# stein7/nerf-navigation

Measured on AMD Instinct MI355X. Metric: ray-samples/sec, Stonehenge-class 800x800 novel-view render, higher is better.
Workload: dtype f16

## Files before the change

### nerf-navigation_amd/csrc/render_fused.hip

```cpp
#include "ngp_mlp.h"
#include "ngp_sh.h"
#include "ngp_field.h"
#include "ngp_march.h"
#include "ngp_camera.h"

__global__ void k_field_forward_lds(rf_params P, const float* __restrict__ xyzs, const float* __restrict__ dirs, uint32_t M,
                                    float* __restrict__ sigmas, void* __restrict__ rgbs, bool rgb_half);

static int rf_field_forward(const ngp_field_t* field_host, const float* xyzs, const float* dirs, uint32_t M, float* sigmas, void* rgbs, bool rgb_half, void* stream) {
    rf_params P;
    int rc = rf_fill_params("field_forward", field_host, P);
    if (rc != NGP_OK) return rc;
    if (M == 0) return NGP_OK;
    NGP_REQUIRE(xyzs && dirs && sigmas && rgbs, "field_forward: null pointer");
    const uint32_t npairs = (M + 31) >> 5;
    uint32_t blocks = ngp_div_up(npairs, RF_BLOCK / 64);
    if (blocks > 256 * RF_FIELD_WG_PER_CU) blocks = 256 * RF_FIELD_WG_PER_CU;
    hipLaunchKernelGGL(k_field_forward_lds, dim3(blocks), dim3(RF_BLOCK), 36 * 1024, (hipStream_t)stream, P, xyzs, dirs, M, sigmas, rgbs, rgb_half);
    NGP_CHECK_LAUNCH("field_forward");
    return NGP_OK;
}

extern "C" int ngp_field_forward(const ngp_field_t* field_host, const float* xyzs, const float* dirs, uint32_t M,
                                 float* sigmas, float* rgbs, void* stream) {
    return rf_field_forward(field_host, xyzs, dirs, M, sigmas, rgbs, false, stream);
}

extern "C" int ngp_field_forward_half(const ngp_field_t* field_host, const float* xyzs, const float* dirs, uint32_t M,
                                      float* sigmas, void* rgbs_half, void* stream) {
    return rf_field_forward(field_host, xyzs, dirs, M, sigmas, rgbs_half, true, stream);
}


#ifndef RV_S
#define RV_S 12
#endif
static_assert(RV_S >= 2, "RV_S must be at least 2: the one-sample-per-round frame kernel has been removed");
#ifndef RV_BANDS
#define RV_BANDS 32u
#endif
#ifndef RV_REFILL_MIN
#define RV_REFILL_MIN 64
#endif
#ifndef RV_SLAB_STEPS
#define RV_SLAB_STEPS 16
#endif
#ifndef RV_BLOCK_THREADS
#define RV_BLOCK_THREADS 512
#endif
#ifndef RV_BLOCKS_PER_CU
#define RV_BLOCKS_PER_CU 1
#endif
static constexpr uint32_t RV_BLOCK = RV_BLOCK_THREADS;
static constexpr int RV_WAVES_PER_SIMD = (RV_BLOCK_THREADS / 256) * RV_BLOCKS_PER_CU;
static constexpr int RV_WAVES = RV_BLOCK / 64;
static constexpr uint32_t RV_LDS_W = RV_NFRAG * 1024;
static constexpr uint32_t RV_LDS_SH = RV_WAVES * 64 * 32;
static constexpr uint32_t RV_LDS_LV = 4 * 96;

struct rf_frame {
    const float* rays_o; const float* rays_d; uint32_t N;
    ngp_camera cam;
    const ngp_camera* cams; uint32_t frame_rays;
    float aabb[6]; float min_near;
    const uint8_t* bitfield; uint32_t C, H;
    float dt_gamma; uint32_t max_steps;
    float bg[3];
    float* image; float* depth; float* weights_sum;
    uint32_t* stats; uint32_t* queue;
#ifdef RV_COUNTERS
    uint32_t* hist;
#endif
    const uint32_t* coarse;
    uint32_t coarse_words;
    uint32_t tile_w;
    uint32_t skip;
    const uint32_t* occ_ext;
    float occ_unit, occ_top;
    const uint32_t* tile_perm;
};

__global__ __launch_bounds__(256) void k_build_coarse(const uint8_t* __restrict__ bitfield, uint32_t n_blocks_total,
                                                      uint32_t* __restrict__ coarse, uint32_t blocks_per_level, uint32_t C, uint32_t* __restrict__ ext) {
    const uint32_t w = blockIdx.x * 256 + threadIdx.x;
    if (w * 32 >= n_blocks_total) return;
    const uint64_t* b64 = reinterpret_cast<const uint64_t*>(bitfield);
    uint32_t bits = 0;
    #pragma unroll 8
    for (uint32_t i = 0; i < 32; i++) {
        const uint32_t blk = w * 32 + i;
        if (blk < n_blocks_total && b64[blk] != 0ull) bits |= 1u << i;
    }
    coarse[w] = bits;
    if (ext && bits) {
        uint32_t nb = 1;
        while (nb * nb * nb < blocks_per_level) nb <<= 1;
        uint32_t lo[3] = {0xFFFFFFFFu, 0xFFFFFFFFu, 0xFFFFFFFFu}, hi[3] = {0u, 0u, 0u};
        const uint32_t words_per_level = blocks_per_level / 32u, level = w / words_per_level;
        ngp_occ_extent_word(bits, w - level * words_per_level, level, C, nb, lo, hi);
        #pragma unroll
        for (int k = 0; k < 3; k++) { atomicMax(ext + k, (1u << 20) - lo[k]); atomicMax(ext + 3 + k, hi[k]); }
    }
}

struct rv_ray { float ox, oy, oz, dx, dy, dz, rdx, rdy, rdz; };
struct rv_consts {
    float bound, rbound, dt_gamma, dt_min, dt_max, rH, H3, Hf, Cf, Hm1;
    const uint8_t* grid;
    __device__ __forceinline__ int mip(int e) const { return (int)fminf(Cf - 1.0f, fmaxf(0.0f, (float)e)); }
};
__device__ __forceinline__ float rv_uniform(float v) {
    return __builtin_bit_cast(float, __builtin_amdgcn_readfirstlane(__builtin_bit_cast(int, v)));
}
struct rv_view : rv_ray, rv_consts {
    __device__ __forceinline__ rv_view(const rv_ray& r, const rv_consts& k) : rv_ray(r), rv_consts(k) {}
};

typedef ngp_point<rv_view> rv_point;

struct rv_block_cache { uint32_t blk = 0xffffffffu, lo = 0, hi = 0; };

struct rv_tested { rv_point r; bool maybe; uint32_t sw; };

__device__ __forceinline__ bool rv_test(const rv_view& m, const uint32_t* __restrict__ lds_coarse, uint32_t coarse_words, rv_block_cache& bc,
                                        float tc, rv_tested& st
#ifdef RV_COUNTERS
                                        , int* rv_dbg_ptr
#endif
                                        ) {
    rv_point& r = st.r;
    r.at(m, tc);
    const uint32_t mort = ngp_morton3((uint32_t)r.nx, (uint32_t)r.ny, (uint32_t)r.nz);
    st.maybe = true;
    st.sw = 0;
    if (lds_coarse) {
        const uint32_t blk = mort >> 6;
        st.maybe = (lds_coarse[(uint32_t)r.level * coarse_words + (blk >> 5)] >> (blk & 31u)) & 1u;
        st.sw = (uint32_t)r.level * coarse_words + ((blk >> 6) << 1);
#ifdef RV_COUNTERS
        *rv_dbg_ptr = st.maybe ? 0 : ((lds_coarse[st.sw] | lds_coarse[st.sw + 1]) == 0u ? 2 : 1);
#endif
    }
    if (!st.maybe) return false;
    if (lds_coarse) {
        const uint32_t gblk = (uint32_t)r.level * (coarse_words << 5) + (mort >> 6);
        if (gblk != bc.blk) {
            const uint2 w = reinterpret_cast<const uint2*>(m.grid)[gblk];
            bc.blk = gblk; bc.lo = w.x; bc.hi = w.y;
        }
        return (((mort & 32u) ? bc.hi : bc.lo) >> (mort & 31u)) & 1u;
    }
    const uint32_t index = (uint32_t)((float)r.level * m.H3 + (float)mort);
    return (m.grid[index >> 3] >> (index & 7u)) & 1u;
}

__device__ __forceinline__ float rv_leave(const rv_view& m, const uint32_t* __restrict__ lds_coarse, float M, const rv_tested& st, float tc) {
    const rv_point& r = st.r;
    const float tt = r.cell_exit(m, tc);
    if (lds_coarse && !st.maybe) {
        const int sh = ((lds_coarse[st.sw] | lds_coarse[st.sw + 1]) == 0u) ? 4 : 2;
        const float ta = ngp_try_skip(m, r, tc, tt, sh, M);
        if (ta >= 0.0f) return ta;
    }
    float tp;
    return ngp_advance(m, tc, tt, tp);
}

__device__ __forceinline__ bool rv_probe(const rv_ray& ray, const rv_consts& k, const uint32_t* __restrict__ lds_coarse, uint32_t coarse_words,
                                         float M, rv_block_cache& bc, float& t, float& x, float& y, float& z, float& dt
#ifdef RV_COUNTERS
                                         , int* rv_dbg_ptr
#endif
                                         ) {
    const rv_view m(ray, k);
    rv_tested st;
#ifdef RV_COUNTERS
    const bool occ = rv_test(m, lds_coarse, coarse_words, bc, t, st, rv_dbg_ptr);
#else
    const bool occ = rv_test(m, lds_coarse, coarse_words, bc, t, st);
#endif
    x = st.r.x; y = st.r.y; z = st.r.z; dt = st.r.dt;
    if (occ) return true;
    t = rv_leave(m, lds_coarse, M, st, t);
    return false;
}


template <bool FIXED>
__device__ __forceinline__ void rf_points_loop(const rf_params& P, const rf_iter_class cls_rt, const rf_lane_levels& lv, const ngp_h8* __restrict__ lds_w,
                                               const float* __restrict__ xyzs, const float* __restrict__ dirs, uint32_t M,
                                               float* __restrict__ sigmas, void* __restrict__ rgbs_v, bool rgb_half) {
    const rf_iter_class cls = FIXED ? rf_iter_class{1u, 12u, 2u} : cls_rt;
    const int lane = threadIdx.x & 63, g = lane >> 4, s = lane & 15;
    const uint32_t wave = (blockIdx.x * RF_BLOCK + threadIdx.x) >> 6, nwaves = gridDim.x * (RF_BLOCK / 64);
    const uint32_t npairs = (M + 31) >> 5;
    for (uint32_t pair = wave; pair < npairs; pair += nwaves) {
        ngp_h8 x[2];
        ngp_h4 shq[2];
        uint32_t m[2];
        #pragma unroll
        for (int n = 0; n < 2; n++) {
            m[n] = pair * 32 + 16 * n + s;
            const uint64_t mm = m[n] < M ? m[n] : 0;
            const float px = xyzs[3 * mm], py = xyzs[3 * mm + 1], pz = xyzs[3 * mm + 2];
            float sh[16];
            sh_eval<4>(dirs[3 * mm], dirs[3 * mm + 1], dirs[3 * mm + 2], P.shn, sh);
            #pragma unroll
            for (int j = 0; j < 4; j++) {
                float v = sh[j];
                if (g == 1) v = sh[4 + j];
                if (g == 2) v = sh[8 + j];
                if (g == 3) v = sh[12 + j];
                shq[n][j] = ngp_f2h(v);
            }
            x[n] = rf_encode<false>(P, lv, cls, px, py, pz);
        }
        float sg[2], cr[2], cg[2], cb[2];
        rv_mlp_tiles<2>(lds_w, lane, x, shq, sg, cr, cg, cb);
        #pragma unroll
        for (int n = 0; n < 2; n++)
            if (g == 0 && m[n] < M) {
                rv_activate(P, sg[n], cr[n], cg[n], cb[n]);
                sigmas[m[n]] = sg[n];
                if (rgb_half) {
                    _Float16* rgbs = static_cast<_Float16*>(rgbs_v);
                    rgbs[3ull * m[n]] = (_Float16)cr[n]; rgbs[3ull * m[n] + 1] = (_Float16)cg[n]; rgbs[3ull * m[n] + 2] = (_Float16)cb[n];
                } else {
                    float* rgbs = static_cast<float*>(rgbs_v);
                    rgbs[3ull * m[n]] = cr[n]; rgbs[3ull * m[n] + 1] = cg[n]; rgbs[3ull * m[n] + 2] = cb[n];
                }
            }
    }
}

__global__ __launch_bounds__(RF_BLOCK, RF_FIELD_WG_PER_CU) void k_field_forward_lds(rf_params P, const float* __restrict__ xyzs, const float* __restrict__ dirs,
                                                                    uint32_t M, float* __restrict__ sigmas, void* __restrict__ rgbs, bool rgb_half) {
    extern __shared__ __attribute__((aligned(16))) unsigned char rf_smem[];
    ngp_h8* lds_w = reinterpret_cast<ngp_h8*>(rf_smem);
    const int lane = threadIdx.x & 63, g = lane >> 4, wave = threadIdx.x >> 6;
    rv_stage_weights(P, lds_w, wave, RF_BLOCK / 64, lane);
    rf_lane_levels lv;
    rf_setup_levels(P, g, lv);
    __syncthreads();
    const rf_iter_class cls = rf_classify(lv);
    if (cls.dense == 1u && cls.select == 2u && cls.hashed == 12u) rf_points_loop<true>(P, cls, lv, lds_w, xyzs, dirs, M, sigmas, rgbs, rgb_half);
    else rf_points_loop<false>(P, cls, lv, lds_w, xyzs, dirs, M, sigmas, rgbs, rgb_half);
}

__device__ __forceinline__ void rv_ray_od(const rf_frame& F, uint32_t ray, float o[3], float d[3]) {
    if (F.rays_o) {
        #pragma unroll
        for (int k = 0; k < 3; k++) { o[k] = F.rays_o[3ull * ray + k]; d[k] = F.rays_d[3ull * ray + k]; }
    } else if (F.cams) {
        const uint32_t f = ray / F.frame_rays;
        const ngp_camera c = F.cams[f];
        o[0] = c.t[0]; o[1] = c.t[1]; o[2] = c.t[2];
        ngp_camera_ray(c, ray - f * F.frame_rays, d);
    } else {
        o[0] = F.cam.t[0]; o[1] = F.cam.t[1]; o[2] = F.cam.t[2];
        ngp_camera_ray(F.cam, ray, d);
    }
}

__device__ __forceinline__ uint32_t rv_ray_of(uint32_t idx, uint32_t tile_w) {
    if (tile_w == 0) return idx;
    const uint32_t tile = idx >> 6, in = idx & 63u, tiles_x = tile_w >> 3;
    const uint32_t ty = tile / tiles_x, tx = tile - ty * tiles_x;
    const uint32_t p = in >> 4, s = in & 15u;
    const uint32_t px = (p & 1u) * 4 + (s & 3u), py = (p >> 1) * 4 + (s >> 2);
    return (ty * 8 + py) * tile_w + tx * 8 + px;
}

static constexpr uint32_t RV_LDS_SMP = RV_WAVES * 64 * RV_S * 16;

template <bool FIXED>
__device__ __forceinline__ void rv_frame_loop(const rf_params& P, const rf_frame& F, const rf_iter_class cls_rt,
                                              const ngp_h8* __restrict__ lds_w, _Float16* lds_sh, const rf_lane_levels* lds_lv,
                                              float4* lds_smp, const uint32_t* lds_coarse, const float* lds_occ) {
    const rf_iter_class cls = FIXED ? rf_iter_class{1u, 12u, 2u} : cls_rt;
    const int lane = threadIdx.x & 63, g = lane >> 4, s = lane & 15, wave = threadIdx.x >> 6;
    const int wave_s = __builtin_amdgcn_readfirstlane(wave);

    _Float16* my_sh = lds_sh + (wave * 64 + lane) * 16;
    const _Float16* wave_sh = lds_sh + wave * 64 * 16;
    float4* my_smp = lds_smp + (wave * 64 + lane) * RV_S;
    float4* wave_smp = lds_smp + wave * 64 * RV_S;

    rv_consts K;
    K.bound = P.bound; K.rbound = rv_uniform(1.0f / P.bound); K.dt_gamma = F.dt_gamma;
    K.Hf = rv_uniform((float)F.H); K.Cf = rv_uniform((float)F.C); K.Hm1 = rv_uniform((float)(F.H - 1));
    K.rH = rv_uniform(1.0f / K.Hf);
    K.H3 = rv_uniform((float)(F.H * F.H * F.H));
    K.dt_min = rv_uniform((2.0f * 1.7320508075688772f) / (float)F.max_steps);
    K.dt_max = rv_uniform(((2.0f * 1.7320508075688772f) * (float)(1 << (F.C - 1))) / K.Hf);
    K.grid = F.bitfield;

    bool active = false;
    uint32_t ray = 0, nsamp = 0;
    rv_ray m;
    float t = 0, last_t = 0, near = 0, far = 0;
    float ws = 0, dacc = 0, cr = 0, cg = 0, cb = 0, tcomp = 0;
    bool exhausted = false;
    uint32_t rv_q = blockIdx.x & 7u, rv_q_seen = 0;
    rv_block_cache bc;
    uint32_t n_samples_local = 0, n_tiles = 0, n_capped_local = 0, n_hit_local = 0;
#ifdef RV_COUNTERS
    uint32_t n_rounds = 0, n_trips = 0, n_probe[4] = {0, 0, 0, 0};
    unsigned long long c_refill = 0, c_march = 0, c_tiles = 0, c_comp = 0;
    const unsigned long long c_start = __builtin_readcyclecounter();
    unsigned long long c_last = c_start;
#define RV_TICK(acc) { const unsigned long long c_now = __builtin_readcyclecounter(); acc += c_now - c_last; c_last = c_now; }
    uint32_t* rv_hist = F.hist;
    unsigned long long rv_t0 = 0;
    if (rv_hist) {
        unsigned long long* p0 = reinterpret_cast<unsigned long long*>(F.queue + 24);
        const unsigned long long now = wall_clock64();
        const unsigned long long old = atomicCAS(p0, 0ull, now);
        rv_t0 = __shfl(old ? old : now, 0, 64);
    }
#else
#define RV_TICK(acc)
#endif

    for (;;) {
        if (!exhausted) {
            const unsigned long long need = __ballot(!active);
            if (need && (uint32_t)__popcll(need) >= RV_REFILL_MIN) {
                const uint32_t cnt = (uint32_t)__popcll(need);
                uint32_t base = 0;
                const uint32_t n_tiles64 = (F.N + 63u) >> 6;
                const uint32_t q_lo = (uint32_t)(((unsigned long long)n_tiles64 * rv_q) / RV_BANDS) << 6;
                uint32_t q_hi = (uint32_t)(((unsigned long long)n_tiles64 * (rv_q + 1u)) / RV_BANDS) << 6;
                q_hi = q_hi < F.N ? q_hi : F.N;
                if (lane == 0) base = atomicAdd(F.queue + 32 + rv_q, cnt);
                base = __shfl(base, 0, 64) + q_lo;
                if (!active) {
                    const uint32_t idx = base + (uint32_t)__popcll(need & ((1ull << lane) - 1ull));
                    if (idx < q_hi) {
                        ray = rv_ray_of(F.tile_perm ? (F.tile_perm[idx >> 6] << 6) | (idx & 63u) : idx, F.tile_w);
                        float o[3], d[3];
                        rv_ray_od(F, ray, o, d);
                        ngp_near_far_inline(o, d, F.aabb, F.min_near, near, far);
                        if (lds_occ) {
                            float n2, f2;
                            ngp_near_far_inline(o, d, lds_occ, 0.0f, n2, f2);
                            far = f2 == 3.402823466e+38f ? near : fminf(far, f2 + lds_occ[6]);
                        }
                        m.ox = o[0]; m.oy = o[1]; m.oz = o[2];
                        m.dx = d[0]; m.dy = d[1]; m.dz = d[2];
                        m.rdx = 1.0f / m.dx; m.rdy = 1.0f / m.dy; m.rdz = 1.0f / m.dz;
                        t = near; last_t = near; tcomp = near;
                        ws = 0; dacc = 0; cr = 0; cg = 0; cb = 0; nsamp = 0;
                        float sh[16];
                        sh_eval<4>(m.dx, m.dy, m.dz, P.shn, sh);
                        #pragma unroll
                        for (int j = 0; j < 16; j++) my_sh[j] = ngp_f2h(sh[j]);
                        active = true;
                    }
                }
                if (base + cnt >= q_hi) {
                    rv_q += 8u;
                    if (rv_q >= RV_BANDS) rv_q = (rv_q + 1u) & 7u;
                    if (++rv_q_seen == RV_BANDS) exhausted = true;
                }
            }
        }
        if (__ballot(active) == 0ull) {
            if (exhausted) break;
            continue;
        }
        RV_TICK(c_refill)

        int cnt = 0;
        bool ended = false;
#ifdef RV_COUNTERS
        n_rounds++;
        const unsigned long long rv_live = __ballot(active);
#endif
        {
            rv_ray mr = m;
            float far_r = far;
            asm("" : "+v"(mr.ox), "+v"(mr.oy), "+v"(mr.oz), "+v"(mr.dx), "+v"(mr.dy), "+v"(mr.dz),
                     "+v"(mr.rdx), "+v"(mr.rdy), "+v"(mr.rdz), "+v"(far_r));
            rv_consts Kr = K;
            asm("" : "+v"(Kr.Hf), "+v"(Kr.Hm1), "+v"(Kr.Cf), "+v"(Kr.rH), "+v"(Kr.dt_min), "+v"(Kr.dt_max), "+v"(Kr.rbound), "+v"(Kr.H3));
            const float M = (active && F.skip) ? ngp_skip_margin(mr, K.bound, lds_occ ? far_r + 4.0f * K.bound : far_r) : __builtin_inff();
            const uint32_t slot0 = ((uint32_t)wave_s * 64u + __builtin_amdgcn_mbcnt_hi(~0u, __builtin_amdgcn_mbcnt_lo(~0u, 0u))) * RV_S;
            float4* const smp_w = lds_smp + slot0;
            int probes = 0;
            float t_lim = __builtin_inff();
            auto march = [&](int upto) {
                for (;;) {
#ifdef RV_COUNTERS
                    n_trips = __builtin_amdgcn_readfirstlane(n_trips) + 1;
#endif
                    if (!(t < far_r && nsamp < F.max_steps)) { ended = true; break; }
                    if (RV_SLAB_STEPS > 0 && !(t < t_lim)) break;
                    float x, y, z, dt;
#ifdef RV_COUNTERS
                    int pc = 0;
                    const bool hit = rv_probe(mr, Kr, lds_coarse, F.coarse_words, M, bc, t, x, y, z, dt, &pc);
                    n_probe[pc]++;
                    if (hit) {
#else
                    if (rv_probe(mr, Kr, lds_coarse, F.coarse_words, M, bc, t, x, y, z, dt)) {
#endif
                        smp_w[cnt] = make_float4(x, y, z, t);
                        t += dt;
                        nsamp++;
                        if (++cnt >= upto) break;
                    }
                    if (++probes >= RF_PROBES_PER_ROUND) break;
                }
            };
            if (RV_SLAB_STEPS > 0) {
                if (active) march(1);
                const float t_first = cnt ? smp_w[0].w : __builtin_inff();
                float tf = t_first;
                #pragma unroll
                for (int off = 1; off < 64; off <<= 1) tf = fminf(tf, __shfl_xor(tf, off, 64));
                t_lim = tf + (float)RV_SLAB_STEPS * K.dt_min;
                if (cnt && !(t_first < t_lim)) { t = t_first; nsamp--; cnt = 0; ended = false; }
                if (active && cnt && !ended) march(RV_S);
            } else if (active) {
                march(RV_S);
            }
        }

        __builtin_amdgcn_fence(__ATOMIC_RELEASE, "wavefront");
        __builtin_amdgcn_wave_barrier();
        __builtin_amdgcn_fence(__ATOMIC_ACQUIRE, "wavefront");

        RV_TICK(c_march)
        int col_src;
        {
            uint32_t rank = 0, above = 0;
            const uint32_t below_me = __builtin_amdgcn_mbcnt_hi(~0u, __builtin_amdgcn_mbcnt_lo(~0u, 0u));
            #pragma unroll
            for (int c = RV_S; c >= 0; c--) {
                const unsigned long long mc = __ballot(cnt == c);
                if (cnt == c) rank = above + (uint32_t)__popcll(mc & ((1ull << below_me) - 1ull));
                above += (uint32_t)__popcll(mc);
            }
            col_src = __builtin_amdgcn_ds_permute((int)(rank << 2), (int)below_me);
        }
        #pragma unroll 1
        for (int p = 0; p < 4; p++) {
            const int src = __shfl(col_src, 16 * p + s, 64);
            const int ccol = __shfl(cnt, src, 64);
            if (__ballot(ccol > 0) == 0ull) continue;
            const ngp_h4 shq = *reinterpret_cast<const ngp_h4*>(wave_sh + src * 16 + 4 * g);
            const rf_lane_levels lv = lds_lv[g];
            #pragma unroll 1
            for (int k = 0; k < RV_S; k += 2) {
                if (__ballot(ccol > k) == 0ull) break;
                if (k + 1 < RV_S && __ballot(ccol > k + 1) != 0ull) {
                    ngp_h8 xs[2];
                    #pragma unroll
                    for (int n = 0; n < 2; n++) {
                        float4 q = wave_smp[src * RV_S + k + n];
                        if (!(ccol > k + n)) q = make_float4(0.f, 0.f, 0.f, 0.f);
                        xs[n] = rf_encode<true>(P, lv, cls, q.x, q.y, q.z);
                    }
                    n_tiles += 2;
                    const ngp_h4 ss[2] = {shq, shq};
                    float a[2], b[2], c[2], d[2];
                    rv_mlp_tiles<2>(lds_w, lane, xs, ss, a, b, c, d);
                    #pragma unroll
                    for (int n = 0; n < 2; n++)
                        if (g == 0 && ccol > k + n) {
                            ngp_h4 r;
                            r[0] = (_Float16)a[n]; r[1] = (_Float16)b[n]; r[2] = (_Float16)c[n]; r[3] = (_Float16)d[n];
                            *reinterpret_cast<ngp_h4*>(&wave_smp[src * RV_S + k + n]) = r;
                        }
                } else {
                    float4 q = wave_smp[src * RV_S + k];
                    if (!(ccol > k)) q = make_float4(0.f, 0.f, 0.f, 0.f);
                    n_tiles++;
                    float a, b, c, d;
                    rv_field_tile(P, lv, cls, lds_w, lane, q.x, q.y, q.z, shq, a, b, c, d);
                    if (g == 0 && ccol > k) {
                        ngp_h4 r;
                        r[0] = (_Float16)a; r[1] = (_Float16)b; r[2] = (_Float16)c; r[3] = (_Float16)d;
                        *reinterpret_cast<ngp_h4*>(&wave_smp[src * RV_S + k]) = r;
                    }
                }
            }
        }

        __builtin_amdgcn_fence(__ATOMIC_RELEASE, "wavefront");
        __builtin_amdgcn_wave_barrier();
        __builtin_amdgcn_fence(__ATOMIC_ACQUIRE, "wavefront");

        RV_TICK(c_tiles)
        bool done = false;
        for (int k = 0; k < cnt; k++) {
            const ngp_h4 r = *reinterpret_cast<const ngp_h4*>(&my_smp[k]);
            const float ts = my_smp[k].w;
            const float dt = ngp_clampf(ts * K.dt_gamma, K.dt_min, K.dt_max);
            const float ta = ts + dt;
            const float d1 = ta - last_t;
            last_t = ta;
            float sig = (float)r[0], sr = (float)r[1], sg = (float)r[2], sb = (float)r[3];
            rv_activate(P, sig, sr, sg, sb);
            n_samples_local++;
            const float alpha = 1.0f - ngp_expf(-sig * dt);
            const float T = 1 - ws;
            const float w = alpha * T;
            ws += w;
            tcomp += d1;
            dacc += w * tcomp;
            cr += w * sr; cg += w * sg; cb += w * sb;
            if ((double)T < 1e-4) {
                done = true;
#ifdef RV_COUNTERS
                n_probe[3] += (uint32_t)(cnt - (k + 1));
#endif
                break;
            }
        }
        float far0 = far;
        if (lds_occ && (done || ended)) {
            const float o3[3] = {m.ox, m.oy, m.oz}, d3[3] = {m.dx, m.dy, m.dz};
            float n0;
            ngp_near_far_inline(o3, d3, F.aabb, F.min_near, n0, far0);
        }
        const bool capped = !done && ended && nsamp >= F.max_steps && t < far0;
        if (ended) done = true;
        if (done) {
            F.image[3ull * ray] = cr + (1 - ws) * F.bg[0];
            F.image[3ull * ray + 1] = cg + (1 - ws) * F.bg[1];
            F.image[3ull * ray + 2] = cb + (1 - ws) * F.bg[2];
            F.depth[ray] = fmaxf(dacc - near, 0.0f) / (far0 - near);
            F.weights_sum[ray] = ws;
            n_capped_local += capped ? 1u : 0u;
            n_hit_local += nsamp > 0 ? 1u : 0u;
            active = false;
        }
        RV_TICK(c_comp)
#ifdef RV_COUNTERS
        if (rv_hist) {
            const unsigned long long now = wall_clock64();
            const uint32_t bin = now > rv_t0 ? (uint32_t)((now - rv_t0) / 2000ull) : 0u;
            uint32_t rs = (uint32_t)cnt;
            #pragma unroll
            for (int off = 32; off > 0; off >>= 1) rs += __shfl_down(rs, off, 64);
            if (lane == 0 && bin < 512u) {
                atomicAdd(rv_hist + bin, rs); atomicAdd(rv_hist + 512 + bin, 1u);
                atomicAdd(rv_hist + 1024 + bin, (uint32_t)__popcll(rv_live));
            }
        }
#endif
    }
#ifdef RV_COUNTERS
    if (rv_hist && lane == 0) {
        const unsigned long long now = wall_clock64();
        const uint32_t bin = now > rv_t0 ? (uint32_t)((now - rv_t0) / 2000ull) : 0u;
        if (bin < 512u) atomicAdd(rv_hist + 1536 + bin, 1u);
    }
#endif
    uint32_t tot = n_samples_local, tot_capped = n_capped_local, tot_hit = n_hit_local;
    #pragma unroll
    for (int off = 32; off > 0; off >>= 1) {
        tot += __shfl_down(tot, off, 64);
        tot_capped += __shfl_down(tot_capped, off, 64);
        tot_hit += __shfl_down(tot_hit, off, 64);
    }
    if (lane == 0 && tot) atomicAdd(F.stats, tot);
    if (lane == 0 && tot_capped) atomicAdd(F.stats + 1, tot_capped);
    if (lane == 0 && tot_hit) atomicAdd(F.stats + 2, tot_hit);
    if (lane == 0 && n_tiles) atomicAdd(F.stats + 3, n_tiles);
#ifdef RV_COUNTERS
    if (lane == 0) { atomicAdd(F.queue + 1, n_rounds); atomicAdd(F.queue + 2, n_trips); }
    atomicAdd(F.queue + 3, n_probe[0]); atomicAdd(F.queue + 4, n_probe[1]); atomicAdd(F.queue + 5, n_probe[2]); atomicAdd(F.queue + 6, n_probe[3]);
    if (lane == 0) {
        unsigned long long* c = reinterpret_cast<unsigned long long*>(F.queue + 8);
        const unsigned long long c_total = __builtin_readcyclecounter() - c_start;
        atomicAdd(c + 0, c_refill); atomicAdd(c + 1, c_march); atomicAdd(c + 2, c_tiles); atomicAdd(c + 3, c_comp);
        atomicAdd(c + 4, c_total); atomicMax(c + 5, c_total); atomicMax(c + 6, ~c_total);
    }
#endif
}

__global__ __launch_bounds__(RV_BLOCK, RV_WAVES_PER_SIMD) void k_render_frame_multi(rf_params P, rf_frame F) {
    extern __shared__ __attribute__((aligned(16))) unsigned char rv_smem[];
    ngp_h8* lds_w = reinterpret_cast<ngp_h8*>(rv_smem);
    _Float16* lds_sh = reinterpret_cast<_Float16*>(rv_smem + RV_LDS_W);
    rf_lane_levels* lds_lv = reinterpret_cast<rf_lane_levels*>(rv_smem + RV_LDS_W + RV_LDS_SH);
    float4* lds_smp = reinterpret_cast<float4*>(rv_smem + RV_LDS_W + RV_LDS_SH + RV_LDS_LV);
    uint32_t* lds_coarse = F.coarse ? reinterpret_cast<uint32_t*>(rv_smem + RV_LDS_W + RV_LDS_SH + RV_LDS_LV + RV_LDS_SMP) : nullptr;

    const int lane = threadIdx.x & 63, g = lane >> 4, s = lane & 15, wave = threadIdx.x >> 6;

    rv_stage_weights(P, lds_w, wave, RV_WAVES, lane);
    if (lds_coarse) {
        const uint32_t nw = F.coarse_words * F.C;
        for (uint32_t i = threadIdx.x; i < nw; i += RV_BLOCK) lds_coarse[i] = F.coarse[i];
    }
    float* lds_occ = (lds_coarse && F.occ_ext) ? reinterpret_cast<float*>(lds_coarse + F.coarse_words * F.C) : nullptr;
    if (lds_occ && threadIdx.x < 3) {
        const uint32_t k = threadIdx.x;
        const uint32_t hi = F.occ_ext[3 + k], lo = (1u << 20) - F.occ_ext[k];
        const bool any = F.occ_ext[3] != 0u;
        lds_occ[k] = any ? -F.occ_top + ((float)lo - 1.0f) * F.occ_unit : 3.0e38f;
        lds_occ[3 + k] = any ? -F.occ_top + ((float)hi + 1.0f) * F.occ_unit : 3.1e38f;
        if (k == 0) lds_occ[6] = 2.0f * (((2.0f * 1.7320508075688772f) * (float)(1 << (F.C - 1))) / (float)F.H);
    }
    if (wave == 0 && s == 0) {
        rf_lane_levels tmp;
        rf_setup_levels(P, g, tmp);
        lds_lv[g] = tmp;
    }
    __syncthreads();
    const rf_iter_class cls = rf_classify(lds_lv[g]);
    if (cls.dense == 1u && cls.select == 2u && cls.hashed == 12u)
        rv_frame_loop<true>(P, F, cls, lds_w, lds_sh, lds_lv, lds_smp, lds_coarse, lds_occ);
    else
        rv_frame_loop<false>(P, F, cls, lds_w, lds_sh, lds_lv, lds_smp, lds_coarse, lds_occ);
}

static constexpr uint32_t RV_ORDER_MAX = 4096;

__global__ __launch_bounds__(256) void k_tile_cost(rf_frame F, float bound, uint32_t n_tiles, uint32_t* __restrict__ cost) {
    const uint32_t tile = blockIdx.x * 4u + (threadIdx.x >> 6), lane = threadIdx.x & 63u;
    if (tile >= n_tiles) return;
    rv_consts K;
    K.bound = bound; K.rbound = 1.0f / bound; K.dt_gamma = F.dt_gamma;
    K.Hf = (float)F.H; K.Cf = (float)F.C; K.Hm1 = (float)(F.H - 1); K.rH = 1.0f / K.Hf; K.H3 = (float)(F.H * F.H * F.H);
    K.dt_min = (2.0f * 1.7320508075688772f) / (float)F.max_steps;
    K.dt_max = ((2.0f * 1.7320508075688772f) * (float)(1 << (F.C - 1))) / K.Hf;
    K.grid = F.bitfield;
    float box[7] = {0.f, 0.f, 0.f, 0.f, 0.f, 0.f, 0.f};
    if (F.occ_ext) {
        const bool any = F.occ_ext[3] != 0u;
        #pragma unroll
        for (int k = 0; k < 3; k++) {
            const uint32_t hi = F.occ_ext[3 + k], lo = (1u << 20) - F.occ_ext[k];
            box[k] = any ? -F.occ_top + ((float)lo - 1.0f) * F.occ_unit : 3.0e38f;
            box[3 + k] = any ? -F.occ_top + ((float)hi + 1.0f) * F.occ_unit : 3.1e38f;
        }
        box[6] = 2.0f * K.dt_max;
    }
    const uint32_t tiles_x = F.tile_w >> 3, ty = tile / tiles_x, tx = tile - ty * tiles_x;
    float acc = 0.0f;
    #pragma unroll
    for (int r = 0; r < 5; r++) {
        const uint32_t px = r == 4 ? 4u : (r & 1) * 7u, py = r == 4 ? 4u : (r >> 1) * 7u;
        float o[3], d[3], near, far;
        rv_ray_od(F, (ty * 8u + py) * F.tile_w + tx * 8u + px, o, d);
        ngp_near_far_inline(o, d, F.aabb, F.min_near, near, far);
        if (F.occ_ext) {
            float n2, f2;
            ngp_near_far_inline(o, d, box, 0.0f, n2, f2);
            far = f2 == 3.402823466e+38f ? near : fminf(far, f2 + box[6]);
        }
        rv_ray m;
        m.ox = o[0]; m.oy = o[1]; m.oz = o[2]; m.dx = d[0]; m.dy = d[1]; m.dz = d[2]; m.rdx = m.rdy = m.rdz = 0.0f;
        const rv_view v(m, K);
        const float seg = far > near ? (far - near) * (1.0f / 64.0f) : 0.0f;
        rv_point pt;
        pt.at(v, (far > near ? near : 0.0f) + ((float)lane + 0.5f) * seg);
        const uint32_t blk = ngp_morton3((uint32_t)pt.nx, (uint32_t)pt.ny, (uint32_t)pt.nz) >> 6;
        if ((F.coarse[(uint32_t)pt.level * F.coarse_words + (blk >> 5)] >> (blk & 31u)) & 1u) acc += seg / pt.dt;
    }
    #pragma unroll
    for (int off = 32; off > 0; off >>= 1) acc += __shfl_xor(acc, off, 64);
    if (lane == 0) cost[tile] = (uint32_t)fminf(acc + 0.5f, 4.0e9f);
}

__global__ __launch_bounds__(1024) void k_tile_sort(const uint32_t* __restrict__ cost, uint32_t n_tiles, uint32_t* __restrict__ perm) {
    __shared__ __attribute__((aligned(16))) uint32_t c[RV_ORDER_MAX];
    const uint32_t b = blockIdx.x;
    const uint32_t lo = (uint32_t)(((unsigned long long)n_tiles * b) / RV_BANDS), hi = (uint32_t)(((unsigned long long)n_tiles * (b + 1u)) / RV_BANDS);
    const uint32_t n = hi - lo, n4 = (n + 3u) & ~3u;
    for (uint32_t i = threadIdx.x; i < n4; i += 1024u) c[i] = i < n ? cost[lo + i] : 0u;
    __syncthreads();
    const uint4* c4 = reinterpret_cast<const uint4*>(c);
    for (uint32_t i = threadIdx.x; i < n; i += 1024u) {
        const uint32_t ci = c[i];
        uint32_t rank = 0;
        #pragma unroll 4
        for (uint32_t j = 0; j < n4; j += 4u) {
            const uint4 q = c4[j >> 2];
            rank += (q.x > ci || (q.x == ci && j < i)) ? 1u : 0u;
            rank += (q.y > ci || (q.y == ci && j + 1u < i)) ? 1u : 0u;
            rank += (q.z > ci || (q.z == ci && j + 2u < i)) ? 1u : 0u;
            rank += (q.w > ci || (q.w == ci && j + 3u < i)) ? 1u : 0u;
        }
        perm[lo + rank] = lo + i;
    }
}

static inline bool rv_pow2(uint32_t v) { return v && !(v & (v - 1)); }

static std::atomic<int> rv_occ_box_enabled{1};
extern "C" int ngp_render_set_occupied_box(int enabled) { return rv_occ_box_enabled.exchange(enabled ? 1 : 0, std::memory_order_relaxed); }
static std::atomic<int> rv_block_skip_enabled{1};
extern "C" int ngp_render_set_block_skip(int enabled) { return rv_block_skip_enabled.exchange(enabled ? 1 : 0, std::memory_order_relaxed); }
static std::atomic<int> rv_tile_order_enabled{1};
extern "C" int ngp_render_set_tile_order(int enabled) { return rv_tile_order_enabled.exchange(enabled ? 1 : 0, std::memory_order_relaxed); }

static constexpr size_t RV_WS_HEADER_WORDS = 64, RV_WS_COARSE_BYTES = 36 * 1024, RV_WS_HIST_WORDS = 2048, RV_WS_HIST_BYTES = 12 * 1024;
static_assert(RV_LDS_W + RV_LDS_SH + RV_LDS_LV + RV_LDS_SMP + RV_WS_COARSE_BYTES > 160 * 1024, "the coarse map could reach the histogram");
static_assert(RV_WS_HIST_WORDS * sizeof(uint32_t) <= RV_WS_HIST_BYTES, "workspace carve");
struct rv_ws {
    uint32_t* header; uint32_t* occ_ext; uint32_t* queues; uint32_t* coarse; uint32_t* hist; uint32_t* perm; uint32_t* cost; size_t frame_total; ngp_camera* cams; size_t total;
};
static rv_ws rv_layout(uint32_t N, uint32_t n_cams, void* base) {
    const size_t n64 = ngp_div_up(N, 64u);
    ngp_carver c(base);
    return {c.take<uint32_t>(26, 1), c.take<uint32_t>(6, 1), c.take<uint32_t>(32, 1), c.take<uint32_t>(RV_WS_COARSE_BYTES / 4, 1), c.take<uint32_t>(RV_WS_HIST_BYTES / 4, 1),
            c.take<uint32_t>(n64, 1), c.take<uint32_t>(n64, 1), c.total(), c.take<ngp_camera>(n_cams), c.total()};
}
static_assert(RV_BANDS <= 32 && 26 + 6 + 32 == RV_WS_HEADER_WORDS, "workspace header");
extern "C" size_t ngp_render_frame_workspace(uint32_t N) { return rv_layout(N, 0, nullptr).frame_total; }

static int rv_fill_camera(const char* who, const float* pose_host, const float* intrinsics_host, uint32_t H, uint32_t W, ngp_camera& cam) {
    NGP_REQUIRE(pose_host && intrinsics_host, "camera: pose / intrinsics are host pointers and must not be null");
    NGP_REQUIRE(H >= 1 && W >= 1 && (uint64_t)H * W <= 0xFFFFFFFFull, "camera: bad image size");
    NGP_REQUIRE(intrinsics_host[0] != 0.0f && intrinsics_host[1] != 0.0f, "camera: zero focal length");
    for (int r = 0; r < 3; r++) {
        for (int c = 0; c < 3; c++) cam.r[3 * r + c] = pose_host[4 * r + c];
        cam.t[r] = pose_host[4 * r + 3];
    }
    cam.fx = intrinsics_host[0]; cam.fy = intrinsics_host[1]; cam.cx = intrinsics_host[2]; cam.cy = intrinsics_host[3];
    cam.W = W; cam.H = H;
    (void)who;
    return NGP_OK;
}

static int rv_render_frame(const ngp_field_t* field_host, const float* rays_o, const float* rays_d, const ngp_camera* cam, uint32_t n_cams, uint32_t N,
                           uint32_t image_width, const float* aabb_host, float min_near, const uint8_t* bitfield, uint32_t C, uint32_t Hgrid,
                           float dt_gamma, uint32_t max_steps, const float* bg_color3_host,
                           float* image, float* depth, float* weights_sum, uint32_t* stats,
                           void* workspace, size_t workspace_bytes, void* stream) {
    rf_params P;
    int rc = rf_fill_params("render_frame", field_host, P);
    if (rc != NGP_OK) return rc;
    const rv_ws ws = rv_layout(N, cam && n_cams > 1 ? n_cams : 0u, workspace);
    NGP_REQUIRE(stats && workspace && ngp_ws_holds(workspace, workspace_bytes, ws.header, RV_WS_HEADER_WORDS * 4), "render_frame: stats / workspace missing");
    NGP_REQUIRE(aabb_host && bg_color3_host, "render_frame: aabb / bg_color are host pointers and must not be null");
    NGP_REQUIRE(C >= 1 && C <= 16 && Hgrid >= 1 && Hgrid <= 1024 && max_steps >= 1, "render_frame: bad C/H/max_steps");
    NGP_REQUIRE(rv_pow2(Hgrid), "render_frame: the grid size must be a power of two (cells are addressed by Morton index)");
    hipStream_t s = (hipStream_t)stream;
    if (hipMemsetAsync(stats, 0, 4 * sizeof(uint32_t), s) != hipSuccess || hipMemsetAsync(ws.header, 0, RV_WS_HEADER_WORDS * 4, s) != hipSuccess)
        return ngp_fail(NGP_ELAUNCH, "render_frame: memset failed");
    if (N == 0) return NGP_OK;
    NGP_REQUIRE((cam || (rays_o && rays_d)) && bitfield && image && depth && weights_sum, "render_frame: null pointer");
    rf_frame F;
    F.rays_o = cam ? nullptr : rays_o; F.rays_d = cam ? nullptr : rays_d; F.N = N;
    F.cam = cam ? *cam : ngp_camera{};
    F.cams = nullptr; F.frame_rays = N;
    if (cam && n_cams > 1) {
        NGP_REQUIRE(workspace_bytes >= ws.total, "render_frames_camera: workspace too small (ngp_render_frames_workspace)");
        ngp_camera* dst = ws.cams;
        if (hipMemcpyAsync(dst, cam, n_cams * sizeof(ngp_camera), hipMemcpyHostToDevice, s) != hipSuccess) return ngp_fail(NGP_ELAUNCH, "render_frames_camera: camera copy failed");
        F.cams = dst; F.frame_rays = N / n_cams;
    }
    for (int i = 0; i < 6; i++) F.aabb[i] = aabb_host[i];
    F.min_near = min_near; F.bitfield = bitfield; F.C = C; F.H = Hgrid;
    F.dt_gamma = dt_gamma; F.max_steps = max_steps;
    for (int i = 0; i < 3; i++) F.bg[i] = bg_color3_host[i];
    F.image = image; F.depth = depth; F.weights_sum = weights_sum;
    F.stats = stats; F.queue = ws.header;
#ifdef RV_COUNTERS
    F.hist = nullptr;
#ifdef RV_TIMELINE
    if (ngp_ws_holds(workspace, workspace_bytes, ws.hist, RV_WS_HIST_WORDS * sizeof(uint32_t))) {
        F.hist = ws.hist;
        if (hipMemsetAsync(F.hist, 0, RV_WS_HIST_WORDS * sizeof(uint32_t), s) != hipSuccess) return ngp_fail(NGP_ELAUNCH, "render_frame: memset failed");
    }
#endif
#endif
    F.tile_w = 0;
    const uint32_t hint = image_width;
    if (hint >= 8 && hint % 8 == 0 && N % hint == 0 && (N / hint) % 8 == 0) F.tile_w = hint;

    F.coarse = nullptr; F.coarse_words = 0; F.skip = 0; F.occ_ext = nullptr; F.occ_unit = 0.0f; F.occ_top = 0.0f;
    F.tile_perm = nullptr;
    static_assert(sizeof(rf_lane_levels) * 4 == RV_LDS_LV, "LDS carve of the level table");
    size_t lds = RV_LDS_W + RV_LDS_SH + RV_LDS_LV + RV_LDS_SMP;
    const uint64_t blocks_per_level = (uint64_t)Hgrid * Hgrid * Hgrid / 64;
    const uint64_t coarse_bytes = (uint64_t)C * blocks_per_level / 8;
    if (rv_pow2(Hgrid) && Hgrid >= 8 && blocks_per_level % 32 == 0 && lds + coarse_bytes <= 160 * 1024 && (uint64_t)C * Hgrid * Hgrid * Hgrid <= (1ull << 24) &&
        ngp_ws_holds(workspace, workspace_bytes, ws.coarse, coarse_bytes) && (reinterpret_cast<uintptr_t>(bitfield) & 7u) == 0) {
        uint32_t* coarse = ws.coarse;
        const uint32_t n_blocks_total = (uint32_t)(C * blocks_per_level);
        F.coarse = coarse;
        F.coarse_words = (uint32_t)(blocks_per_level / 32);
        lds += coarse_bytes;
        uint32_t* ext = nullptr;
        const bool nested = ngp_skip_allowed(C, Hgrid, field_host->bound);
        if (nested && rv_occ_box_enabled.load(std::memory_order_relaxed) && lds + 32 <= 160 * 1024) {
            ext = ws.occ_ext;
            F.occ_ext = ext;
            F.occ_top = C == 1 ? field_host->bound : (float)(1u << (C - 1));
            F.occ_unit = 2.0f * (C == 1 ? field_host->bound : 1.0f) / (float)(Hgrid / 4);
            lds += 32;
        }
        hipLaunchKernelGGL(k_build_coarse, dim3(ngp_div_up(n_blocks_total / 32, 256)), dim3(256), 0, s, bitfield, n_blocks_total, coarse,
                           (uint32_t)blocks_per_level, C, ext);
        F.skip = (rv_block_skip_enabled.load(std::memory_order_relaxed) && nested) ? 1u : 0u;
    }
    const uint32_t n_tiles = F.tile_w ? N / 64u : 0u;
    if (n_tiles && !F.cams && F.coarse && rv_tile_order_enabled.load(std::memory_order_relaxed) && ngp_div_up(n_tiles, RV_BANDS) <= RV_ORDER_MAX &&
        workspace_bytes >= ws.frame_total) {
        uint32_t* perm = ws.perm;
        uint32_t* cost = ws.cost;
        hipLaunchKernelGGL(k_tile_cost, dim3(ngp_div_up(n_tiles, 4u)), dim3(256), 0, s, F, P.bound, n_tiles, cost);
        hipLaunchKernelGGL(k_tile_sort, dim3(RV_BANDS), dim3(1024), 0, s, cost, n_tiles, perm);
        NGP_CHECK_LAUNCH("render_frame: tile order");
        F.tile_perm = perm;
    }
    NGP_REQUIRE(lds <= 160 * 1024, "render_frame: LDS carve exceeds 160 KiB");
    static std::atomic<unsigned long long> attr_devices{0};
    const int rc_lds = ngp_allow_dynamic_lds(attr_devices, {reinterpret_cast<const void*>(k_render_frame_multi)}, 160 * 1024);
    if (rc_lds == NGP_LDS_NO_DEVICE) return ngp_fail(NGP_ELAUNCH, "render_frame: no current device");
    if (rc_lds != NGP_LDS_OK) return ngp_fail(NGP_ELAUNCH, "render_frame: cannot raise the dynamic LDS limit");
    uint32_t blocks = 256 * RV_BLOCKS_PER_CU;
    const uint32_t need = ngp_div_up(N, RV_BLOCK);
    if (blocks > need) blocks = need;
    hipLaunchKernelGGL(k_render_frame_multi, dim3(blocks), dim3(RV_BLOCK), lds, s, P, F);
    NGP_CHECK_LAUNCH("render_frame");
    return NGP_OK;
}

extern "C" int ngp_render_frame(const ngp_field_t* field_host, const float* rays_o, const float* rays_d, uint32_t N,
                                uint32_t image_width, const float* aabb_host, float min_near, const uint8_t* bitfield, uint32_t C, uint32_t Hgrid,
                                float dt_gamma, uint32_t max_steps, const float* bg_color3_host,
                                float* image, float* depth, float* weights_sum, uint32_t* stats,
                                void* workspace, size_t workspace_bytes, void* stream) {
    return rv_render_frame(field_host, rays_o, rays_d, nullptr, 0, N, image_width, aabb_host, min_near, bitfield, C, Hgrid, dt_gamma, max_steps,
                           bg_color3_host, image, depth, weights_sum, stats, workspace, workspace_bytes, stream);
}

extern "C" int ngp_render_frame_camera(const ngp_field_t* field_host, const float* pose_host, const float* intrinsics_host, uint32_t H, uint32_t W,
                                       const float* aabb_host, float min_near, const uint8_t* bitfield, uint32_t C, uint32_t Hgrid,
                                       float dt_gamma, uint32_t max_steps, const float* bg_color3_host,
                                       float* image, float* depth, float* weights_sum, uint32_t* stats,
                                       void* workspace, size_t workspace_bytes, void* stream) {
    ngp_camera cam;
    const int rc = rv_fill_camera("render_frame_camera", pose_host, intrinsics_host, H, W, cam);
    if (rc != NGP_OK) return rc;
    return rv_render_frame(field_host, nullptr, nullptr, &cam, 1, H * W, W, aabb_host, min_near, bitfield, C, Hgrid, dt_gamma, max_steps,
                           bg_color3_host, image, depth, weights_sum, stats, workspace, workspace_bytes, stream);
}

extern "C" size_t ngp_render_frames_workspace(uint32_t P, uint32_t rays_per_frame) { return rv_layout(P * rays_per_frame, P, nullptr).total; }

extern "C" int ngp_render_frames_camera(const ngp_field_t* field_host, const float* poses_host, uint32_t P, const float* intrinsics_host, uint32_t H, uint32_t W,
                                        const float* aabb_host, float min_near, const uint8_t* bitfield, uint32_t C, uint32_t Hgrid,
                                        float dt_gamma, uint32_t max_steps, const float* bg_color3_host,
                                        float* image, float* depth, float* weights_sum, uint32_t* stats,
                                        void* workspace, size_t workspace_bytes, void* stream) {
    NGP_REQUIRE(P >= 1 && P <= 64, "render_frames_camera: 1..64 frames per launch");
    NGP_REQUIRE(H % 8 == 0 && W % 8 == 0, "render_frames_camera: H and W must be multiples of 8");
    NGP_REQUIRE((uint64_t)P * H * W <= 0xFFFFFFFFull, "render_frames_camera: too many rays");
    NGP_REQUIRE(poses_host, "render_frames_camera: poses is a host pointer and must not be null");
    ngp_camera cams[64];
    for (uint32_t p = 0; p < P; p++) {
        const int rc = rv_fill_camera("render_frames_camera", poses_host + 16 * p, intrinsics_host, H, W, cams[p]);
        if (rc != NGP_OK) return rc;
    }
    return rv_render_frame(field_host, nullptr, nullptr, cams, P, P * H * W, W, aabb_host, min_near, bitfield, C, Hgrid, dt_gamma, max_steps,
                           bg_color3_host, image, depth, weights_sum, stats, workspace, workspace_bytes, stream);
}

__global__ __launch_bounds__(256) void k_get_rays(ngp_camera cam, const int64_t* __restrict__ inds, uint32_t N,
                                                  float* __restrict__ rays_o, float* __restrict__ rays_d) {
    const uint32_t k = blockIdx.x * 256 + threadIdx.x;
    if (k >= N) return;
    uint32_t pixel = k;
    if (inds) {
        const int64_t p = inds[k];
        const int64_t last = (int64_t)cam.W * cam.H - 1;
        pixel = (uint32_t)(p < 0 ? 0 : p > last ? last : p);
    }
    float d[3];
    ngp_camera_ray(cam, pixel, d);
    #pragma unroll
    for (int c = 0; c < 3; c++) { rays_o[3ull * k + c] = cam.t[c]; rays_d[3ull * k + c] = d[c]; }
}

extern "C" int ngp_get_rays(const float* pose_host, const float* intrinsics_host, uint32_t H, uint32_t W,
                            const int64_t* inds, uint32_t N, float* rays_o, float* rays_d, void* stream) {
    ngp_camera cam;
    const int rc = rv_fill_camera("get_rays", pose_host, intrinsics_host, H, W, cam);
    if (rc != NGP_OK) return rc;
    if (N == 0) return NGP_OK;
    NGP_REQUIRE(inds || (uint64_t)N == (uint64_t)H * W, "get_rays: N must be H * W when inds is null");
    NGP_REQUIRE(rays_o && rays_d, "get_rays: null pointer");
    hipLaunchKernelGGL(k_get_rays, dim3(ngp_div_up(N, 256u)), dim3(256), 0, (hipStream_t)stream, cam, inds, N, rays_o, rays_d);
    NGP_CHECK_LAUNCH("get_rays");
    return NGP_OK;
}
```

Measured before the change: 9.450 billion.

## Fuse frame memsets, coarse-map build and tile costing into one prologue kernel

Replaces two memsets, the coarse occupancy build kernel and the tile cost kernel with a single prologue kernel. Each workgroup rebuilds the coarse bitmap in LDS using wave ballots and reduces the occupancy extent without global atomics. Tile costing then reads LDS instead of global memory and broadcasts each ray's setup across lanes with readlane. This removes launch and dependency overhead before the render kernel. The cost is that every workgroup redundantly scans the whole bitfield, and the header and stats are now zeroed from inside the kernel.

```diff
diff --git a/nerf-navigation_amd/csrc/render_fused.hip b/nerf-navigation_amd/csrc/render_fused.hip
--- a/nerf-navigation_amd/csrc/render_fused.hip
+++ b/nerf-navigation_amd/csrc/render_fused.hip
@@ -1,3 +1,4 @@
+#include <algorithm>
 #include "ngp_mlp.h"
 #include "ngp_sh.h"
 #include "ngp_field.h"
@@ -79,29 +80,6 @@
     float occ_unit, occ_top;
     const uint32_t* tile_perm;
 };
-
-__global__ __launch_bounds__(256) void k_build_coarse(const uint8_t* __restrict__ bitfield, uint32_t n_blocks_total,
-                                                      uint32_t* __restrict__ coarse, uint32_t blocks_per_level, uint32_t C, uint32_t* __restrict__ ext) {
-    const uint32_t w = blockIdx.x * 256 + threadIdx.x;
-    if (w * 32 >= n_blocks_total) return;
-    const uint64_t* b64 = reinterpret_cast<const uint64_t*>(bitfield);
-    uint32_t bits = 0;
-    #pragma unroll 8
-    for (uint32_t i = 0; i < 32; i++) {
-        const uint32_t blk = w * 32 + i;
-        if (blk < n_blocks_total && b64[blk] != 0ull) bits |= 1u << i;
-    }
-    coarse[w] = bits;
-    if (ext && bits) {
-        uint32_t nb = 1;
-        while (nb * nb * nb < blocks_per_level) nb <<= 1;
-        uint32_t lo[3] = {0xFFFFFFFFu, 0xFFFFFFFFu, 0xFFFFFFFFu}, hi[3] = {0u, 0u, 0u};
-        const uint32_t words_per_level = blocks_per_level / 32u, level = w / words_per_level;
-        ngp_occ_extent_word(bits, w - level * words_per_level, level, C, nb, lo, hi);
-        #pragma unroll
-        for (int k = 0; k < 3; k++) { atomicMax(ext + k, (1u << 20) - lo[k]); atomicMax(ext + 3 + k, hi[k]); }
-    }
-}
 
 struct rv_ray { float ox, oy, oz, dx, dy, dz, rdx, rdy, rdz; };
 struct rv_consts {
@@ -620,55 +598,146 @@
 }
 
 static constexpr uint32_t RV_ORDER_MAX = 4096;
-
-__global__ __launch_bounds__(256) void k_tile_cost(rf_frame F, float bound, uint32_t n_tiles, uint32_t* __restrict__ cost) {
-    const uint32_t tile = blockIdx.x * 4u + (threadIdx.x >> 6), lane = threadIdx.x & 63u;
-    if (tile >= n_tiles) return;
+static constexpr uint32_t RV_PRO_MAP_BYTES = 160 * 1024 - (RV_LDS_W + RV_LDS_SH + RV_LDS_LV + RV_LDS_SMP);
+static constexpr uint32_t RV_PRO_RUN = 12;
+static_assert(RV_PRO_MAP_BYTES % 4 == 0 && RV_PRO_MAP_BYTES + 1024 <= 64 * 1024 && 5 * RV_PRO_RUN <= 64, "k_frame_prologue");
+
+struct rv_pro {
+    uint32_t* stats; uint32_t* header;
+    uint32_t n_blocks_total, blocks_per_level;
+    uint32_t* coarse; uint32_t* ext;
+    uint32_t n_tiles, run; uint32_t* cost;
+    float bound;
+};
+
+__device__ __forceinline__ float rv_lane_f(float v, uint32_t src) {
+    return __builtin_bit_cast(float, __builtin_amdgcn_readlane(__builtin_bit_cast(int, v), (int)src));
+}
+
+__global__ __launch_bounds__(1024) void k_frame_prologue(rf_frame F, rv_pro Q) {
+    __shared__ uint32_t map[RV_PRO_MAP_BYTES / 4];
+    __shared__ uint32_t red[16][6];
+    __shared__ uint32_t ext[6];
+    const uint32_t tid = threadIdx.x, lane = tid & 63u, wave = (uint32_t)__builtin_amdgcn_readfirstlane((int)(tid >> 6));
+    const bool first = blockIdx.x == 0;
+
+    if (Q.n_blocks_total) {
+        const uint2* b64 = reinterpret_cast<const uint2*>(F.bitfield);
+        for (uint32_t base = wave * 512u; base < Q.n_blocks_total; base += 16u * 512u) {
+            uint2 v[8];
+            #pragma unroll
+            for (uint32_t j = 0; j < 8; j++) {
+                const uint32_t blk = base + j * 64u + lane;
+                v[j] = blk < Q.n_blocks_total ? b64[blk] : make_uint2(0u, 0u);
+            }
+            #pragma unroll
+            for (uint32_t j = 0; j < 8; j++) {
+                const unsigned long long m = __ballot((v[j].x | v[j].y) != 0u);
+                const uint32_t w = ((base + j * 64u) >> 5) + lane;
+                if (lane < 2u && w * 32u < Q.n_blocks_total) {
+                    const uint32_t bits = lane ? (uint32_t)(m >> 32) : (uint32_t)m;
+                    map[w] = bits;
+                    if (first) Q.coarse[w] = bits;
+                }
+            }
+        }
+        __syncthreads();
+        if (Q.ext) {
+            uint32_t nb = 1;
+            while (nb * nb * nb < Q.blocks_per_level) nb <<= 1;
+            uint32_t lo[3] = {0xFFFFFFFFu, 0xFFFFFFFFu, 0xFFFFFFFFu}, hi[3] = {0u, 0u, 0u};
+            const uint32_t words_per_level = Q.blocks_per_level / 32u, n_words = Q.n_blocks_total / 32u;
+            for (uint32_t w = tid; w < n_words; w += 1024u) {
+                const uint32_t level = w / words_per_level;
+                ngp_occ_extent_word(map[w], w - level * words_per_level, level, F.C, nb, lo, hi);
+            }
+            #pragma unroll
+            for (int k = 0; k < 3; k++) {
+                #pragma unroll
+                for (int off = 32; off > 0; off >>= 1) {
+                    const uint32_t l2 = __shfl_xor(lo[k], off, 64), h2 = __shfl_xor(hi[k], off, 64);
+                    lo[k] = l2 < lo[k] ? l2 : lo[k];
+                    hi[k] = h2 > hi[k] ? h2 : hi[k];
+                }
+                if (lane == 0) { red[wave][k] = lo[k]; red[wave][3 + k] = hi[k]; }
+            }
+            __syncthreads();
+            if (tid < 6u) {
+                uint32_t r = red[0][tid];
+                for (uint32_t i = 1; i < 16u; i++) r = tid < 3u ? (red[i][tid] < r ? red[i][tid] : r) : (red[i][tid] > r ? red[i][tid] : r);
+                uint32_t any = red[0][3];
+                for (uint32_t i = 1; i < 16u; i++) any |= red[i][3];
+                ext[tid] = !any ? 0u : tid < 3u ? (1u << 20) - r : r;
+            }
+            __syncthreads();
+        }
+    }
+    if (first) {
+        if (tid < 64u) Q.header[tid] = (Q.n_blocks_total && Q.ext && tid >= 26u && tid < 32u) ? ext[tid - 26u] : 0u;
+        else if (tid < 68u) Q.stats[tid - 64u] = 0u;
+    }
+    if (!Q.n_tiles) return;
+
     rv_consts K;
-    K.bound = bound; K.rbound = 1.0f / bound; K.dt_gamma = F.dt_gamma;
+    K.bound = Q.bound; K.rbound = 1.0f / Q.bound; K.dt_gamma = F.dt_gamma;
     K.Hf = (float)F.H; K.Cf = (float)F.C; K.Hm1 = (float)(F.H - 1); K.rH = 1.0f / K.Hf; K.H3 = (float)(F.H * F.H * F.H);
     K.dt_min = (2.0f * 1.7320508075688772f) / (float)F.max_steps;
     K.dt_max = ((2.0f * 1.7320508075688772f) * (float)(1 << (F.C - 1))) / K.Hf;
     K.grid = F.bitfield;
     float box[7] = {0.f, 0.f, 0.f, 0.f, 0.f, 0.f, 0.f};
     if (F.occ_ext) {
-        const bool any = F.occ_ext[3] != 0u;
+        const bool any = ext[3] != 0u;
         #pragma unroll
         for (int k = 0; k < 3; k++) {
-            const uint32_t hi = F.occ_ext[3 + k], lo = (1u << 20) - F.occ_ext[k];
+            const uint32_t hi = ext[3 + k], lo = (1u << 20) - ext[k];
             box[k] = any ? -F.occ_top + ((float)lo - 1.0f) * F.occ_unit : 3.0e38f;
             box[3 + k] = any ? -F.occ_top + ((float)hi + 1.0f) * F.occ_unit : 3.1e38f;
         }
         box[6] = 2.0f * K.dt_max;
     }
-    const uint32_t tiles_x = F.tile_w >> 3, ty = tile / tiles_x, tx = tile - ty * tiles_x;
-    float acc = 0.0f;
-    #pragma unroll
-    for (int r = 0; r < 5; r++) {
-        const uint32_t px = r == 4 ? 4u : (r & 1) * 7u, py = r == 4 ? 4u : (r >> 1) * 7u;
-        float o[3], d[3], near, far;
-        rv_ray_od(F, (ty * 8u + py) * F.tile_w + tx * 8u + px, o, d);
-        ngp_near_far_inline(o, d, F.aabb, F.min_near, near, far);
-        if (F.occ_ext) {
-            float n2, f2;
-            ngp_near_far_inline(o, d, box, 0.0f, n2, f2);
-            far = f2 == 3.402823466e+38f ? near : fminf(far, f2 + box[6]);
-        }
-        rv_ray m;
-        m.ox = o[0]; m.oy = o[1]; m.oz = o[2]; m.dx = d[0]; m.dy = d[1]; m.dz = d[2]; m.rdx = m.rdy = m.rdz = 0.0f;
-        const rv_view v(m, K);
-        const float seg = far > near ? (far - near) * (1.0f / 64.0f) : 0.0f;
-        rv_point pt;
-        pt.at(v, (far > near ? near : 0.0f) + ((float)lane + 0.5f) * seg);
-        const uint32_t blk = ngp_morton3((uint32_t)pt.nx, (uint32_t)pt.ny, (uint32_t)pt.nz) >> 6;
-        if ((F.coarse[(uint32_t)pt.level * F.coarse_words + (blk >> 5)] >> (blk & 31u)) & 1u) acc += seg / pt.dt;
-    }
-    #pragma unroll
-    for (int off = 32; off > 0; off >>= 1) acc += __shfl_xor(acc, off, 64);
-    if (lane == 0) cost[tile] = (uint32_t)fminf(acc + 0.5f, 4.0e9f);
-}
-
-__global__ __launch_bounds__(1024) void k_tile_sort(const uint32_t* __restrict__ cost, uint32_t n_tiles, uint32_t* __restrict__ perm) {
+    const uint32_t tiles_x = F.tile_w >> 3;
+    for (uint32_t i0 = (blockIdx.x * 16u + wave) * Q.run; i0 < Q.n_tiles; i0 += gridDim.x * 16u * Q.run) {
+        const uint32_t lk = lane / 5u, lr = lane - lk * 5u;
+        float o[3] = {0.f, 0.f, 0.f}, d[3] = {0.f, 0.f, 0.f}, t0 = 0.0f, seg = 0.0f;
+        if (lk < Q.run && i0 + lk < Q.n_tiles) {
+            const uint32_t tile = i0 + lk, ty = tile / tiles_x, tx = tile - ty * tiles_x;
+            const uint32_t px = lr == 4u ? 4u : (lr & 1u) * 7u, py = lr == 4u ? 4u : (lr >> 1) * 7u;
+            float near, far;
+            rv_ray_od(F, (ty * 8u + py) * F.tile_w + tx * 8u + px, o, d);
+            ngp_near_far_inline(o, d, F.aabb, F.min_near, near, far);
+            if (F.occ_ext) {
+                float n2, f2;
+                ngp_near_far_inline(o, d, box, 0.0f, n2, f2);
+                far = f2 == 3.402823466e+38f ? near : fminf(far, f2 + box[6]);
+            }
+            seg = far > near ? (far - near) * (1.0f / 64.0f) : 0.0f;
+            t0 = far > near ? near : 0.0f;
+        }
+        const uint32_t nk = Q.n_tiles - i0 < Q.run ? Q.n_tiles - i0 : Q.run;
+        for (uint32_t k = 0; k < nk; k++) {
+            float acc = 0.0f;
+            #pragma unroll
+            for (uint32_t r = 0; r < 5u; r++) {
+                const uint32_t src = 5u * k + r;
+                rv_ray m;
+                m.ox = rv_lane_f(o[0], src); m.oy = rv_lane_f(o[1], src); m.oz = rv_lane_f(o[2], src);
+                m.dx = rv_lane_f(d[0], src); m.dy = rv_lane_f(d[1], src); m.dz = rv_lane_f(d[2], src);
+                m.rdx = m.rdy = m.rdz = 0.0f;
+                const float sg = rv_lane_f(seg, src);
+                const rv_view v(m, K);
+                rv_point pt;
+                pt.at(v, rv_lane_f(t0, src) + ((float)lane + 0.5f) * sg);
+                const uint32_t blk = ngp_morton3((uint32_t)pt.nx, (uint32_t)pt.ny, (uint32_t)pt.nz) >> 6;
+                if ((map[(uint32_t)pt.level * F.coarse_words + (blk >> 5)] >> (blk & 31u)) & 1u) acc += sg / pt.dt;
+            }
+            #pragma unroll
+            for (int off = 32; off > 0; off >>= 1) acc += __shfl_xor(acc, off, 64);
+            if (lane == 0) Q.cost[i0 + k] = (uint32_t)fminf(acc + 0.5f, 4.0e9f);
+        }
+    }
+}
+
+__global__ __launch_bounds__(1024) void k_tile_rank(const uint32_t* __restrict__ cost, uint32_t n_tiles, uint32_t* __restrict__ perm) {
     __shared__ __attribute__((aligned(16))) uint32_t c[RV_ORDER_MAX];
     const uint32_t b = blockIdx.x;
     const uint32_t lo = (uint32_t)(((unsigned long long)n_tiles * b) / RV_BANDS), hi = (uint32_t)(((unsigned long long)n_tiles * (b + 1u)) / RV_BANDS);
@@ -743,9 +812,14 @@
     NGP_REQUIRE(C >= 1 && C <= 16 && Hgrid >= 1 && Hgrid <= 1024 && max_steps >= 1, "render_frame: bad C/H/max_steps");
     NGP_REQUIRE(rv_pow2(Hgrid), "render_frame: the grid size must be a power of two (cells are addressed by Morton index)");
     hipStream_t s = (hipStream_t)stream;
-    if (hipMemsetAsync(stats, 0, 4 * sizeof(uint32_t), s) != hipSuccess || hipMemsetAsync(ws.header, 0, RV_WS_HEADER_WORDS * 4, s) != hipSuccess)
-        return ngp_fail(NGP_ELAUNCH, "render_frame: memset failed");
-    if (N == 0) return NGP_OK;
+    rv_pro Q;
+    Q.stats = stats; Q.header = ws.header; Q.n_blocks_total = 0; Q.blocks_per_level = 0; Q.coarse = nullptr; Q.ext = nullptr;
+    Q.n_tiles = 0; Q.run = 1; Q.cost = nullptr; Q.bound = P.bound;
+    if (N == 0) {
+        hipLaunchKernelGGL(k_frame_prologue, dim3(1), dim3(1024), 0, s, rf_frame{}, Q);
+        NGP_CHECK_LAUNCH("render_frame: prologue");
+        return NGP_OK;
+    }
     NGP_REQUIRE((cam || (rays_o && rays_d)) && bitfield && image && depth && weights_sum, "render_frame: null pointer");
     rf_frame F;
     F.rays_o = cam ? nullptr : rays_o; F.rays_d = cam ? nullptr : rays_d; F.N = N;
@@ -798,20 +872,20 @@
             F.occ_unit = 2.0f * (C == 1 ? field_host->bound : 1.0f) / (float)(Hgrid / 4);
             lds += 32;
         }
-        hipLaunchKernelGGL(k_build_coarse, dim3(ngp_div_up(n_blocks_total / 32, 256)), dim3(256), 0, s, bitfield, n_blocks_total, coarse,
-                           (uint32_t)blocks_per_level, C, ext);
+        Q.n_blocks_total = n_blocks_total; Q.blocks_per_level = (uint32_t)blocks_per_level; Q.coarse = coarse; Q.ext = ext;
         F.skip = (rv_block_skip_enabled.load(std::memory_order_relaxed) && nested) ? 1u : 0u;
     }
     const uint32_t n_tiles = F.tile_w ? N / 64u : 0u;
     if (n_tiles && !F.cams && F.coarse && rv_tile_order_enabled.load(std::memory_order_relaxed) && ngp_div_up(n_tiles, RV_BANDS) <= RV_ORDER_MAX &&
         workspace_bytes >= ws.frame_total) {
-        uint32_t* perm = ws.perm;
-        uint32_t* cost = ws.cost;
-        hipLaunchKernelGGL(k_tile_cost, dim3(ngp_div_up(n_tiles, 4u)), dim3(256), 0, s, F, P.bound, n_tiles, cost);
-        hipLaunchKernelGGL(k_tile_sort, dim3(RV_BANDS), dim3(1024), 0, s, cost, n_tiles, perm);
-        NGP_CHECK_LAUNCH("render_frame: tile order");
-        F.tile_perm = perm;
-    }
+        Q.n_tiles = n_tiles; Q.cost = ws.cost;
+        F.tile_perm = ws.perm;
+    }
+    const uint32_t pro_wgs = Q.n_tiles ? std::min(256u, ngp_div_up(Q.n_tiles, 16u)) : 1u;
+    Q.run = Q.n_tiles ? std::min(RV_PRO_RUN, ngp_div_up(Q.n_tiles, pro_wgs * 16u)) : 1u;
+    hipLaunchKernelGGL(k_frame_prologue, dim3(pro_wgs), dim3(1024), 0, s, F, Q);
+    if (Q.n_tiles) hipLaunchKernelGGL(k_tile_rank, dim3(RV_BANDS), dim3(1024), 0, s, Q.cost, Q.n_tiles, ws.perm);
+    NGP_CHECK_LAUNCH("render_frame: prologue");
     NGP_REQUIRE(lds <= 160 * 1024, "render_frame: LDS carve exceeds 160 KiB");
     static std::atomic<unsigned long long> attr_devices{0};
     const int rc_lds = ngp_allow_dynamic_lds(attr_devices, {reinterpret_cast<const void*>(k_render_frame_multi)}, 160 * 1024);
```

Result: no change. 9.490 billion (median of 6 runs) (+0.4%).
